# QI2lab/ray_trace_pb

Measured on NVIDIA B200. Metric: ray_surfaces_per_s_fp64, higher is better.
Workload: dtype f64

## Files before the change

ray_trace_pb_b200/csrc/rtb_device.cuh:

```cuda
#pragma once

#include <cstdint>
#include <cuda_runtime.h>

#include "../../include/rtb.h"

namespace rtb {

constexpr int kMaxSurfaces = RTB_MAX_SURFACES;
constexpr int kMaxMedia = RTB_MAX_SURFACES + 1;
constexpr int kMaxWavelengths = RTB_MAX_WAVELENGTHS;
constexpr int kMaxSlabs = 2 * RTB_MAX_SURFACES + 1;

#ifndef RTB_TRACE_THREADS
#define RTB_TRACE_THREADS 128
#endif
constexpr int kTraceThreads = RTB_TRACE_THREADS;
#ifndef RTB_TRACE_MIN_BLOCKS
#define RTB_TRACE_MIN_BLOCKS 7
#endif
constexpr int kTraceMinBlocks = RTB_TRACE_MIN_BLOCKS;

struct DevSurface {
    double cx, cy, cz;
    double nx, ny, nz;
    double ax, ay, az;
    double radius, radius_sq, abs_radius;
    double aperture;
    double focal_len;
    double nfx, nfy, nfz;
    double sin_alpha;
    double ap_sq_max;
    double on_sq_lo, on_sq_hi;
    int32_t kind;
    int8_t z_normal;
    int8_t z_axis;
    int8_t degenerate_hint;
    int8_t pad;
};

struct DevMaterial {
    double b0, b1, b2;
    double c0, c1, c2;
    double n_const;
    int32_t kind;
    int32_t pad;
};

struct DevReduce {
    double ox, oy, oz;
    double e1x, e1y, e1z;
    double e2x, e2y, e2z;
    double phase_ref;
    double half_width;
    double inv_cell;
    double *stats;
    double *grid;
    int32_t slab;
    int32_t grid_n;
    double *grid_sin;
    double *grid_count;
    double grid_n_f;
};

__host__ __device__ inline void finish_reduce(DevReduce &r)
{
    const long long plane = (long long)r.grid_n * r.grid_n;
    r.grid_sin = r.grid ? r.grid + plane : nullptr;
    r.grid_count = r.grid ? r.grid + 2 * plane : nullptr;
    r.grid_n_f = (double)r.grid_n;
}

struct DevSource {
    double a_start, a_step, a_stop;
    double b_start, b_step, b_stop;
    double px, py, pz;
    double axx, axy, axz;
    double e1x, e1y, e1z;
    double e2x, e2y, e2z;
    double wavelength;
    long long n_a, n_b;
    long long first;
    int32_t kind;
    int32_t pad;
};

struct TraceParams {
    const double *rays_in;
    double *out;
    long long n_rays;
    long long out_stride;
    int32_t n_surf;
    int32_t n_wl;
    int32_t store_last_only;
    int32_t any_store;
    int32_t flags;
    int32_t pad0;
    int16_t slab_pos[kMaxSlabs + 3];
    uint8_t slab_act[kMaxSurfaces];
    DevReduce red;
    DevSource src;
    const DevSource *src_list;
    int32_t n_src;
    int32_t pad1;
    const unsigned *lean_counts;
    unsigned long long lean_general;
    long long lean_probe_stride;
    long long lean_probe_total;
    int32_t lean_n_runs;
    int32_t lean_sample_run;
    int32_t lean_pure;
    int32_t lean_pad;
    uint8_t lean_run_end[kMaxSurfaces + 2];
    uint8_t lean_run_code[kMaxSurfaces + 2];
    DevSurface surf[kMaxSurfaces];
    DevMaterial mat[kMaxMedia];
    double wl[kMaxWavelengths];
    double n_tab[(kMaxWavelengths + 1) * kMaxMedia];
    double ratio_tab[(kMaxWavelengths + 1) * kMaxMedia];
};

static_assert(sizeof(TraceParams) < 32764, "TraceParams must fit the kernel parameter space");

__device__ __forceinline__ void ld256_stream(const double *p, double &a, double &b, double &c, double &d)
{
    asm volatile("ld.global.nc.L1::no_allocate.v4.f64 {%0,%1,%2,%3}, [%4];"
                 : "=d"(a), "=d"(b), "=d"(c), "=d"(d)
                 : "l"(p));
}

__device__ __forceinline__ void st256(double *p, double a, double b, double c, double d)
{
    asm volatile("st.global.v4.f64 [%0], {%1,%2,%3,%4};" ::"l"(p), "d"(a), "d"(b), "d"(c), "d"(d) : "memory");
}

}
```

ray_trace_pb_b200/csrc/trace_lean.cu:

```cuda
#include <cmath>
#include <math_constants.h>

#include "exact_math.cuh"
#include "lean_steps.cuh"
#include "rtb_device.cuh"
#include "surface_steps.cuh"
#include "trace_common.cuh"

namespace rtb {

namespace {

#ifndef RTB_LEAN_THREADS
#define RTB_LEAN_THREADS 128
#endif
#ifndef RTB_LEAN_MIN_BLOCKS
#define RTB_LEAN_MIN_BLOCKS 7
#endif
constexpr int kLeanThreads = RTB_LEAN_THREADS;
constexpr int kLeanMinBlocks = RTB_LEAN_MIN_BLOCKS;
constexpr int kProbeRays = 2048;
constexpr unsigned kProbeOneIn = 200;

enum StepCode : int { kLeanSphere = 0, kLeanFlat = 1, kGeneralRefracting = 2, kGeneralMirror = 3, kGeneralLens = 4,
                      kMixedRun = 5, kLeanFlatAny = 6, kLeanLens = 7, kLeanFlatZ = 8 };

__host__ __device__ inline int step_code(const DevSurface &s, bool general)
{
    const int fallback = (s.kind == RTB_SURF_MIRROR) ? kGeneralMirror
                                                     : (s.kind == RTB_SURF_PERFECT_LENS) ? kGeneralLens : kGeneralRefracting;
    if (s.kind == RTB_SURF_FLAT && s.z_axis != 0 && s.z_normal != 0) return general ? kLeanFlatZ : kLeanFlat;
    if (general) return fallback;
    if (s.kind == RTB_SURF_SPHERE) return s.z_axis != 0 ? kLeanSphere : fallback;
    if (s.kind == RTB_SURF_FLAT) return kLeanFlatAny;
    if (s.kind == RTB_SURF_PERFECT_LENS) return kLeanLens;
    return fallback;
}

__host__ __device__ inline bool has_lean_step(const DevSurface &s) { return step_code(s, false) < kGeneralRefracting || step_code(s, false) > kMixedRun; }

struct __align__(16) SurfaceShared {
    double rcp;
    int code;
    int rcp_ok;
};

struct LeanShared {
    SurfaceShared surf[kMaxSurfaces];
    int run_clean[kMaxSurfaces + 2];
};

template <bool USE_TABLE>
static __device__ __noinline__ void redo_ray(const TraceParams *P, Ray cur, int k_sample, bool sample_at, Ray *final_row,
                                             Ray *sample_row)
{
    const int n_med = P->n_surf + 1;
    const double wl0 = cur.wl;
    int row = 0;
    bool unlisted = false;
    if (USE_TABLE) {
        row = P->n_wl;
        const long long bits = __double_as_longlong(wl0);
        for (int k = 0; k < P->n_wl; k++)
            if (__double_as_longlong(P->wl[k]) == bits) row = k;
        unlisted = (row == P->n_wl) && (wl0 == wl0);
        row *= n_med;
    }
    auto index_of = [&](int medium) {
        return !USE_TABLE ? eval_index(P->mat[medium], wl0)
                          : (unlisted ? index_for_unlisted(&P->mat[medium], wl0) : P->n_tab[row + medium]);
    };
    double n1 = index_of(0);
    bool dead = false;
    Ray blank;
    set_nan(blank);
    *sample_row = blank;
    for (int k = 0; k < P->n_surf; k++) {
        if (!dead) {
            const DevSurface *s = &P->surf[k];
            const double n2 = index_of(k + 1);
            StepResult res;
            if (s->kind == RTB_SURF_FLAT || s->kind == RTB_SURF_SPHERE) {
                const double ratio = (USE_TABLE && !unlisted) ? P->ratio_tab[row + k] : xm::div(n1, n2);
                res = careful_refracting(s, cur, n1, ratio, true);
            } else if (s->kind == RTB_SURF_MIRROR) {
                res = careful_mirror(s, cur, n1);
            } else {
                res = careful_lens(s, cur, n1, n2, false);
            }
            if (k == k_sample && sample_at) *sample_row = res.at;
            cur = res.after;
            dead = res.dead;
            n1 = n2;
        }
        if (k == k_sample && !sample_at) *sample_row = dead ? blank : cur;
    }
    *final_row = dead ? blank : cur;
}

__device__ __forceinline__ void accumulate(const DevReduce &R, double ox, double oy, double oz, double phase, double *tally)
{
    const double px = ox - R.ox, py = oy - R.oy, pz = oz - R.oz;
    const double u = dot3(px, py, pz, R.e1x, R.e1y, R.e1z);
    const double v = dot3(px, py, pz, R.e2x, R.e2y, R.e2z);
    const double ph = phase - R.phase_ref;
    if (!(isfinite(u) && isfinite(v) && isfinite(ph))) return;
    if (R.stats) {
        double2 *t = reinterpret_cast<double2 *>(tally) + threadIdx.x;
        constexpr int W = kLeanThreads;
        double2 a = t[0 * W], b = t[1 * W], c = t[2 * W], d = t[3 * W], e = t[4 * W], f = t[5 * W];
        a.x += 1.0;
        a.y += u;
        b.x += v;
        b.y += u * u;
        c.x += v * v;
        c.y += u * v;
        d.x += ph;
        d.y += ph * ph;
        e.x = u < e.x ? u : e.x;
        e.y = u > e.y ? u : e.y;
        f.x = v < f.x ? v : f.x;
        f.y = v > f.y ? v : f.y;
        t[0 * W] = a; t[1 * W] = b; t[2 * W] = c; t[3 * W] = d; t[4 * W] = e; t[5 * W] = f;
    }
    if (R.grid) {
        const double xu = (u + R.half_width) * R.inv_cell;
        const double xv = (v + R.half_width) * R.inv_cell;
        const double g = R.grid_n_f;
        if (xu >= 0.0 && xu < g && xv >= 0.0 && xv < g) {
            const unsigned cell = (unsigned)__double2int_rz(xv) * (unsigned)R.grid_n + (unsigned)__double2int_rz(xu);
            double s, c;
            sincos(ph, &s, &c);
            asm volatile("red.global.add.f64 [%0], %1;" ::"l"(R.grid + cell), "d"(c) : "memory");
            asm volatile("red.global.add.f64 [%0], %1;" ::"l"(R.grid_sin + cell), "d"(s) : "memory");
            asm volatile("red.global.add.f64 [%0], %1;" ::"l"(R.grid_count + cell), "d"(1.0) : "memory");
        }
    }
}

__device__ __forceinline__ int tally_index(int k, int thread) { return ((k >> 1) * kLeanThreads + thread) * 2 + (k & 1); }

__device__ __noinline__ void flush_tally(const DevReduce &R, const double *tally)
{
    if (!R.stats) return;
    __shared__ double part[12][kLeanThreads / 32];
    const int lane = threadIdx.x & 31, warp = threadIdx.x >> 5;
    for (int k = 0; k < 12; k++) {
        double x = tally[tally_index(k, threadIdx.x)];
        x = (k < 8) ? warp_sum(x) : ((k == 8 || k == 10) ? warp_min(x) : warp_max(x));
        if (lane == 0) part[k][warp] = x;
    }
    __syncthreads();
    if (threadIdx.x < 12) {
        const int k = threadIdx.x;
        double x = part[k][0];
        for (int w = 1; w < kLeanThreads / 32; w++)
            x = (k < 8) ? x + part[k][w] : ((k == 8 || k == 10) ? fmin(x, part[k][w]) : fmax(x, part[k][w]));
        if (k < 8) {
            if (x != 0.0) atomicAdd(R.stats + k, x);
        } else if (k == 8 || k == 10) {
            if (x < CUDART_INF) atomic_min_f64(R.stats + k, x);
        } else {
            if (x > -CUDART_INF) atomic_max_f64(R.stats + k, x);
        }
    }
}

__device__ __forceinline__ bool general_step(const DevSurface &s, int code, double rcp_y, bool rcp_ok, lean::State &r, double n1,
                                             double n2, double ratio, double wl0, double wl_rcp, bool &ok, bool &kill)
{
    OptimisticZ m;
    xm::Rcp rcp_wl, rcp_k;
    rcp_wl.b = wl0; rcp_wl.y = wl_rcp; rcp_wl.ok = true;
    rcp_k.b = (code == kGeneralLens) ? s.focal_len : s.radius;
    rcp_k.y = rcp_y;
    rcp_k.ok = rcp_ok;
    Ray in, after;
    in.ox = r.ox; in.oy = r.oy; in.oz = r.oz; in.dx = r.dx; in.dy = r.dy; in.dz = r.dz; in.ph = r.ph;
    in.wl = wl0;
    AtRaw raw;
    bool dead;
    if (code == kGeneralRefracting)
        dead = refracting_step<OptimisticZ, true>(m, s, in, n1, ratio, rcp_wl, rcp_k, true, raw, after);
    else if (code == kGeneralMirror)
        dead = mirror_step<OptimisticZ, true>(m, s, in, n1, rcp_wl, raw, after);
    else
        dead = perfect_lens_step<OptimisticZ>(m, s, in, n1, n2, rcp_wl, rcp_k, false, false, raw, after);
    ok = m.ok;
    kill = raw.kill;
    r.ox = after.ox; r.oy = after.oy; r.oz = after.oz;
    r.dx = after.dx; r.dy = after.dy; r.dz = after.dz;
    r.ph = after.ph;
    return !dead;
}

template <bool USE_TABLE, bool FROM_SOURCE, bool SWEEP, bool PROBE, int KINDS>
__global__ void __launch_bounds__(kLeanThreads, kLeanMinBlocks) trace_lean_kernel(const __grid_constant__ TraceParams P,
                                                                                  unsigned *probe_counts)
{
    static_assert(!SWEEP || FROM_SOURCE, "sweeps generate their rays");
    extern __shared__ __align__(16) double s_dyn[];
    const int n_med = P.n_surf + 1;
    double *const s_pair = s_dyn;
    double *const s_tally = s_dyn + (USE_TABLE ? 2 * (P.n_wl + 1) * n_med : 0);
    __shared__ LeanShared s_c;
    __shared__ SweepShared<SWEEP> s_sweep;
    if (SWEEP) sweep_setup(P, s_sweep);
    if (USE_TABLE) {
        const int count = (P.n_wl + 1) * n_med;
        for (int k = threadIdx.x; k < count; k += blockDim.x) {
            s_pair[2 * k] = P.n_tab[k];
            s_pair[2 * k + 1] = P.ratio_tab[k];
        }
    }
    const bool reducing = !PROBE && P.red.slab >= 0;
    if (reducing && P.red.stats) {
        for (int k = 0; k < 12; k++)
            s_tally[tally_index(k, threadIdx.x)] = (k < 8) ? 0.0 : ((k == 8 || k == 10) ? CUDART_INF : -CUDART_INF);
    }
    for (int k = threadIdx.x; k < P.n_surf; k += blockDim.x) {
        const DevSurface &s = P.surf[k];
        const double den = (s.kind == RTB_SURF_PERFECT_LENS) ? s.focal_len : s.radius;
        const double rcp = xm::refine_rcp(den);
        const bool sane = xm::den_ok(den) && fabs(den) < 4503599627370496.0 && xm::quo_ok(rcp);
        s_c.surf[k].rcp = rcp;
        s_c.surf[k].rcp_ok = sane;
        bool general = ((P.lean_general >> k) & 1ull) != 0 ||
                       (!sane && (s.kind == RTB_SURF_SPHERE || s.kind == RTB_SURF_PERFECT_LENS));
        if (!PROBE && KINDS < 2 && P.lean_counts) {
            const unsigned *cnt = P.lean_counts + ((size_t)(SWEEP ? blockIdx.y : 0) * kMaxSurfaces + k) * 2;
            general |= (unsigned long long)cnt[1] * kProbeOneIn > (unsigned long long)cnt[0];
        }
        s_c.surf[k].code = step_code(s, general);
    }
    __syncthreads();
    for (int run = threadIdx.x; KINDS < 2 && run < P.lean_n_runs; run += blockDim.x) {
        bool clean = true;
        for (int k = run > 0 ? P.lean_run_end[run - 1] : 0; k < P.lean_run_end[run]; k++)
            clean &= s_c.surf[k].code == P.lean_run_code[run];
        s_c.run_clean[run] = clean;
    }
    __syncthreads();

    const DevSource &source = sweep_source(P, s_sweep);
    const DevReduce &red = sweep_reduce(P, s_sweep);
    const long long row0 = SWEEP ? (long long)blockIdx.y * P.n_rays : 0;
    const int k_red = reducing ? ((P.red.slab - 1) >> 1) : -1;
    const bool sample_at = reducing && (P.red.slab & 1) != 0;
    const bool planes_in = (P.flags & RTB_FLAG_PLANES_IN) != 0, planes_out = (P.flags & RTB_FLAG_PLANES_OUT) != 0;
    const long long out_rows = P.out_stride / 8;
    const long long stride = (long long)gridDim.x * blockDim.x;
    unsigned *const my_counts = PROBE ? probe_counts + (size_t)(SWEEP ? blockIdx.y : 0) * kMaxSurfaces * 2 : nullptr;

    for (long long base = (long long)blockIdx.x * blockDim.x; base < P.n_rays; base += stride) {
        long long i = base + threadIdx.x;
        const bool valid = i < P.n_rays;
        if (PROBE) {
            const long long st = P.lean_probe_stride;
            i = i * st + (long long)((unsigned)(i * 2654435761u) % (unsigned long long)st);
            if (i >= P.lean_probe_total) i = P.lean_probe_total - 1;
        }
        Ray cur;
        set_nan(cur);
        if (valid) {
            if (FROM_SOURCE)
                cur = make_ray(source, source.first + i);
            else
                load_ray(P.rays_in, i, PROBE ? P.lean_probe_total : P.n_rays, planes_in, cur);
        }
        const double wl0 = cur.wl;
        const double wl_rcp = xm::refine_rcp(wl0);
        int row = 0;
        bool listed = true;
        if (USE_TABLE) {
            row = P.n_wl;
            const long long bits = __double_as_longlong(wl0);
#pragma unroll 1
            for (int k = 0; k < P.n_wl; k++)
                if (__double_as_longlong(P.wl[k]) == bits) row = k;
            listed = row != P.n_wl;
        }
        const double *pair = s_pair + 2 * row * n_med;
        auto non_finite = [](double v) { return (__double2hiint(v) & 0x7ff00000) == 0x7ff00000; };
        const unsigned wl_exp = ((unsigned)__double2hiint(wl0) >> 20) & 0x7ffu;
        const bool fit = valid && listed && (wl_exp - 923u <= 200u) &&
                         !(non_finite(cur.ox) | non_finite(cur.oy) | non_finite(cur.oz) | non_finite(cur.dx) |
                           non_finite(cur.dy) | non_finite(cur.dz) | non_finite(cur.ph));
        bool failed = valid && !fit;
        bool alive = fit;
        bool sampled = false, at_valid = false;
        lean::State r = {cur.ox, cur.oy, cur.oz, cur.dx, cur.dy, cur.dz, cur.ph};
        double n1 = 0.0;
        if (!USE_TABLE) n1 = eval_index(P.mat[0], wl0);

        if (!PROBE) {
            for (int run = 0; run < P.lean_n_runs; run++) {
                const int begin = run > 0 ? P.lean_run_end[run - 1] : 0;
                const int end = P.lean_run_end[run];
                const int code = (KINDS >= 2 || s_c.run_clean[run]) ? P.lean_run_code[run] : kMixedRun;
                if (code == kLeanSphere) {
                    for (int k = begin; k < end; k++) {
                        if (!__any_sync(0xffffffffu, alive)) {
                            at_valid = false;
                            break;
                        }
                        if (USE_TABLE) {
                            n1 = pair[0];
                            pair += 2;
                        }
                        const double n2 = USE_TABLE ? 0.0 : eval_index(P.mat[k + 1], wl0);
                        const double ratio = USE_TABLE ? pair[-1] : xm::div(n1, n2);
                        bool ok = true, kill;
                        const bool on = lean::sphere_axial(ok, P.surf[k], s_c.surf[k].rcp, r, n1, ratio, wl0, wl_rcp, kill);
                        failed = failed | (alive & !ok);
                        at_valid = alive & ok & !kill;
                        alive = alive & ok & on;
                        if (!USE_TABLE) n1 = n2;
                    }
                } else if (code == kLeanFlat) {
                    for (int k = begin; k < end; k++) {
                        if (!__any_sync(0xffffffffu, alive)) {
                            at_valid = false;
                            break;
                        }
                        if (USE_TABLE) {
                            n1 = pair[0];
                            pair += 2;
                        }
                        const double n2 = USE_TABLE ? 0.0 : eval_index(P.mat[k + 1], wl0);
                        const double ratio = USE_TABLE ? pair[-1] : xm::div(n1, n2);
                        bool ok = true, kill;
                        const bool on = lean::flat_axial<false>(ok, P.surf[k], r, n1, ratio, wl0, wl_rcp, kill);
                        failed = failed | (alive & !ok);
                        at_valid = alive & ok & !kill;
                        alive = alive & ok & on;
                        if (!USE_TABLE) n1 = n2;
                    }
                } else if (KINDS >= 2 && code == kLeanFlatZ) {
                    for (int k = begin; k < end; k++) {
                        if (!__any_sync(0xffffffffu, alive)) {
                            at_valid = false;
                            break;
                        }
                        if (USE_TABLE) {
                            n1 = pair[0];
                            pair += 2;
                        }
                        const double n2 = USE_TABLE ? 0.0 : eval_index(P.mat[k + 1], wl0);
                        const double ratio = USE_TABLE ? pair[-1] : xm::div(n1, n2);
                        bool ok = true, kill;
                        const bool on = lean::flat_axial<true>(ok, P.surf[k], r, n1, ratio, wl0, wl_rcp, kill);
                        failed = failed | (alive & !ok);
                        at_valid = alive & ok & !kill;
                        alive = alive & ok & on;
                        if (!USE_TABLE) n1 = n2;
                    }
                } else if ((KINDS == 1 || KINDS == 3) && code == kLeanFlatAny) {
                    for (int k = begin; k < end; k++) {
                        if (!__any_sync(0xffffffffu, alive)) {
                            at_valid = false;
                            break;
                        }
                        if (USE_TABLE) {
                            n1 = pair[0];
                            pair += 2;
                        }
                        const double n2 = USE_TABLE ? 0.0 : eval_index(P.mat[k + 1], wl0);
                        const double ratio = USE_TABLE ? pair[-1] : xm::div(n1, n2);
                        bool ok = true, kill;
                        const bool on = lean::flat_any(ok, P.surf[k], r, n1, ratio, wl0, wl_rcp, kill);
                        failed = failed | (alive & !ok);
                        at_valid = alive & ok & !kill;
                        alive = alive & ok & on;
                        if (!USE_TABLE) n1 = n2;
                    }
                } else if ((KINDS == 1 || KINDS == 3) && code == kLeanLens) {
                    for (int k = begin; k < end; k++) {
                        if (!__any_sync(0xffffffffu, alive)) {
                            at_valid = false;
                            break;
                        }
                        double n2;
                        if (USE_TABLE) {
                            n1 = pair[0];
                            n2 = pair[2];
                            pair += 2;
                        } else {
                            n2 = eval_index(P.mat[k + 1], wl0);
                        }
                        bool ok = true;
                        const bool on = lean::lens_any(ok, P.surf[k], s_c.surf[k].rcp, r, n1, n2, wl0, wl_rcp);
                        failed = failed | (alive & !ok);
                        at_valid = false;
                        alive = alive & ok & on;
                        if (!USE_TABLE) n1 = n2;
                    }
                } else if (KINDS == 1 && code == kGeneralLens) {
                    for (int k = begin; k < end; k++) {
                        if (!__any_sync(0xffffffffu, alive)) {
                            at_valid = false;
                            break;
                        }
                        const DevSurface &s = P.surf[k];
                        const SurfaceShared ss = s_c.surf[k];
                        double ratio, n2;
                        if (USE_TABLE) {
                            n1 = pair[0];
                            ratio = pair[1];
                            n2 = pair[2];
                            pair += 2;
                        } else {
                            n2 = eval_index(P.mat[k + 1], wl0);
                            ratio = xm::div(n1, n2);
                        }
                        bool ok = true, kill;
                        const bool on = general_step(s, kGeneralLens, ss.rcp, ss.rcp_ok != 0, r, n1, n2, ratio, wl0, wl_rcp, ok, kill);
                        failed = failed | (alive & !ok);
                        at_valid = alive & ok & !kill;
                        alive = alive & ok & on;
                        if (!USE_TABLE) n1 = n2;
                    }
                } else if (KINDS < 2 && code == kGeneralRefracting) {
                    for (int k = begin; k < end; k++) {
                        if (!__any_sync(0xffffffffu, alive)) {
                            at_valid = false;
                            break;
                        }
                        const DevSurface &s = P.surf[k];
                        const SurfaceShared ss = s_c.surf[k];
                        double ratio, n2 = 0.0;
                        if (USE_TABLE) {
                            n1 = pair[0];
                            ratio = pair[1];
                            pair += 2;
                        } else {
                            n2 = eval_index(P.mat[k + 1], wl0);
                            ratio = xm::div(n1, n2);
                        }
                        bool ok = true, kill;
                        const bool on = general_step(s, kGeneralRefracting, ss.rcp, ss.rcp_ok != 0, r, n1, n2, ratio, wl0, wl_rcp, ok, kill);
                        failed = failed | (alive & !ok);
                        at_valid = alive & ok & !kill;
                        alive = alive & ok & on;
                        if (!USE_TABLE) n1 = n2;
                    }
                } else if (KINDS < 2) {
                    for (int k = begin; k < end; k++) {
                        if (!__any_sync(0xffffffffu, alive)) {
                            at_valid = false;
                            break;
                        }
                        const DevSurface &s = P.surf[k];
                        const SurfaceShared ss = s_c.surf[k];
                        double ratio, n2 = 0.0;
                        if (USE_TABLE) {
                            n1 = pair[0];
                            ratio = pair[1];
                            n2 = pair[2];
                            pair += 2;
                        } else {
                            n2 = eval_index(P.mat[k + 1], wl0);
                            ratio = xm::div(n1, n2);
                        }
                        bool ok = true, kill;
                        bool on;
                        if (ss.code == kLeanSphere) {
                            on = lean::sphere_axial(ok, s, ss.rcp, r, n1, ratio, wl0, wl_rcp, kill);
                        } else if (ss.code == kLeanFlat) {
                            on = lean::flat_axial<false>(ok, s, r, n1, ratio, wl0, wl_rcp, kill);
                        } else if (ss.code == kLeanFlatZ) {
                            on = lean::flat_axial<true>(ok, s, r, n1, ratio, wl0, wl_rcp, kill);
                        } else if (KINDS == 1 && ss.code == kLeanFlatAny) {
                            on = lean::flat_any(ok, s, r, n1, ratio, wl0, wl_rcp, kill);
                        } else if (KINDS == 1 && ss.code == kLeanLens) {
                            on = lean::lens_any(ok, s, ss.rcp, r, n1, n2, wl0, wl_rcp);
                            kill = false;
                        } else {
                            on = general_step(s, KINDS == 1 ? ss.code : (int)kGeneralRefracting, ss.rcp, ss.rcp_ok != 0, r, n1,
                                              n2, ratio, wl0, wl_rcp, ok, kill);
                        }
                        failed = failed | (alive & !ok);
                        at_valid = alive & ok & !kill;
                        alive = alive & ok & on;
                        if (!USE_TABLE) n1 = n2;
                    }
                }
                if (run == P.lean_sample_run && (sample_at ? at_valid : alive)) {
                    accumulate(red, r.ox, r.oy, r.oz, r.ph, s_tally);
                    sampled = true;
                }
            }
        } else {
            for (int k = 0; k < P.n_surf; k++) {
                if (!alive) break;
                const DevSurface &s = P.surf[k];
                const SurfaceShared ss = s_c.surf[k];
                const int code = ss.code;
                double ratio, n2;
                if (USE_TABLE) {
                    n1 = pair[0];
                    ratio = pair[1];
                    n2 = pair[2];
                    pair += 2;
                } else {
                    n2 = eval_index(P.mat[k + 1], wl0);
                    ratio = xm::div(n1, n2);
                }
                const lean::State before = r;
                bool ok = true, on, kill;
                if (code == kLeanSphere)
                    on = lean::sphere_axial(ok, s, ss.rcp, r, n1, ratio, wl0, wl_rcp, kill);
                else if (code == kLeanFlat)
                    on = lean::flat_axial<false>(ok, s, r, n1, ratio, wl0, wl_rcp, kill);
                else if (code == kLeanFlatZ)
                    on = lean::flat_axial<true>(ok, s, r, n1, ratio, wl0, wl_rcp, kill);
                else if (code == kLeanFlatAny)
                    on = lean::flat_any(ok, s, r, n1, ratio, wl0, wl_rcp, kill);
                else if (code == kLeanLens)
                    on = lean::lens_any(ok, s, ss.rcp, r, n1, n2, wl0, wl_rcp);
                else
                    on = general_step(s, code, ss.rcp, ss.rcp_ok != 0, r, n1, n2, ratio, wl0, wl_rcp, ok, kill);
                atomicAdd(my_counts + 2 * k, 1u);
                if (!ok) {
                    atomicAdd(my_counts + 2 * k + 1, 1u);
                    Ray in;
                    in.ox = before.ox; in.oy = before.oy; in.oz = before.oz;
                    in.dx = before.dx; in.dy = before.dy; in.dz = before.dz;
                    in.ph = before.ph; in.wl = wl0;
                    StepResult res;
                    if (s.kind == RTB_SURF_FLAT || s.kind == RTB_SURF_SPHERE)
                        res = careful_refracting(&s, in, n1, ratio, true);
                    else if (s.kind == RTB_SURF_MIRROR)
                        res = careful_mirror(&s, in, n1);
                    else
                        res = careful_lens(&s, in, n1, n2, false);
                    r.ox = res.after.ox; r.oy = res.after.oy; r.oz = res.after.oz;
                    r.dx = res.after.dx; r.dy = res.after.dy; r.dz = res.after.dz;
                    r.ph = res.after.ph;
                    on = !res.dead;
                }
                alive = on;
                if (!USE_TABLE) n1 = n2;
            }
        }
        if (PROBE) continue;

        Ray out;
        out.ox = r.ox; out.oy = r.oy; out.oz = r.oz; out.dx = r.dx; out.dy = r.dy; out.dz = r.dz; out.ph = r.ph;
        out.wl = wl0;
        if (!alive) set_nan(out);
        if (failed) {
            Ray launch, sample, redone;
            if (FROM_SOURCE)
                launch = make_ray(source, source.first + i);
            else
                load_ray(P.rays_in, i, P.n_rays, planes_in, launch);
            redo_ray<USE_TABLE>(&P, launch, k_red, sample_at, &redone, &sample);
            out = redone;
            if (reducing && !sampled) accumulate(red, sample.ox, sample.oy, sample.oz, sample.ph, s_tally);
        }
        if (valid && P.any_store) store_ray(P.out, row0 + i, out_rows, planes_out, out);
    }
    if (reducing) flush_tally(red, s_tally);
}

bool refracting_only(const TraceParams &P)
{
    for (int k = 0; k < P.n_surf; k++) {
        const DevSurface &s = P.surf[k];
        if (!(s.kind == RTB_SURF_SPHERE || (s.kind == RTB_SURF_FLAT && s.z_axis != 0 && s.z_normal != 0))) return false;
    }
    return true;
}

template <bool T, bool S, bool W, bool PR>
cudaError_t launch_lean_one(const TraceParams &P, unsigned blocks, unsigned n_y, unsigned *probe_counts, cudaStream_t stream)
{
    size_t dyn = T ? 2 * sizeof(double) * (size_t)(P.n_wl + 1) * (size_t)(P.n_surf + 1) : 0;
    if (!PR && P.red.slab >= 0 && P.red.stats) dyn += sizeof(double) * 12 * kLeanThreads;
    const bool pure = !PR && P.lean_pure != 0;
    static const bool loaded = [] {
        cudaFuncAttributes a;
        cudaFuncGetAttributes(&a, trace_lean_kernel<T, S, W, false, 0>);
        cudaFuncGetAttributes(&a, trace_lean_kernel<T, S, W, false, 1>);
        cudaFuncGetAttributes(&a, trace_lean_kernel<T, S, W, false, 2>);
        cudaFuncGetAttributes(&a, trace_lean_kernel<T, S, W, false, 3>);
        cudaFuncGetAttributes(&a, trace_lean_kernel<T, S, W, true, 1>);
        cudaGetLastError();
        return true;
    }();
    (void)loaded;
    if (pure && refracting_only(P))
        trace_lean_kernel<T, S, W, false, 2><<<dim3(blocks, n_y), kLeanThreads, dyn, stream>>>(P, probe_counts);
    else if (pure)
        trace_lean_kernel<T, S, W, false, 3><<<dim3(blocks, n_y), kLeanThreads, dyn, stream>>>(P, probe_counts);
    else if (!PR && refracting_only(P))
        trace_lean_kernel<T, S, W, PR, 0><<<dim3(blocks, n_y), kLeanThreads, dyn, stream>>>(P, probe_counts);
    else
        trace_lean_kernel<T, S, W, PR, 1><<<dim3(blocks, n_y), kLeanThreads, dyn, stream>>>(P, probe_counts);
    return cudaGetLastError();
}

template <bool PR>
cudaError_t launch_lean_pick(const TraceParams &P, unsigned blocks, unsigned *probe_counts, cudaStream_t stream)
{
    const bool table = P.n_wl > 0, source = P.src.kind >= 0, sweep = P.n_src > 0;
    const unsigned n_y = sweep ? (unsigned)P.n_src : 1u;
#ifdef RTB_LEAN_ONLY_ONE
    return launch_lean_one<true, false, false, PR>(P, blocks, 1, probe_counts, stream);
#endif
    if (sweep)
        return table ? launch_lean_one<true, true, true, PR>(P, blocks, n_y, probe_counts, stream)
                     : launch_lean_one<false, true, true, PR>(P, blocks, n_y, probe_counts, stream);
    if (table)
        return source ? launch_lean_one<true, true, false, PR>(P, blocks, 1, probe_counts, stream)
                      : launch_lean_one<true, false, false, PR>(P, blocks, 1, probe_counts, stream);
    return source ? launch_lean_one<false, true, false, PR>(P, blocks, 1, probe_counts, stream)
                  : launch_lean_one<false, false, false, PR>(P, blocks, 1, probe_counts, stream);
}

}

int g_lean_min_share_pct = 75;
void set_lean_min_share_pct(int pct) { g_lean_min_share_pct = pct; }

bool lean_eligible(const TraceParams &P)
{
    if (P.flags & RTB_FLAG_INTERSECT_ONLY) return false;
    if (P.any_store && !P.store_last_only) return false;
    if (P.red.slab == 0) return false;
    if (P.red.slab > 0 && (P.red.slab & 1) != 0 && P.surf[(P.red.slab - 1) >> 1].kind == RTB_SURF_PERFECT_LENS) return false;
    int n_lean = 0;
    for (int k = 0; k < P.n_surf; k++) {
        const DevSurface &s = P.surf[k];
        n_lean += has_lean_step(s);
    }
    if (100 * n_lean < g_lean_min_share_pct * P.n_surf) return false;
    if (P.red.slab < 0 && !P.any_store) return false;
    return P.n_surf > 0;
}

unsigned long long lean_verdict_from_counts(const unsigned *counts, int n_src, int n_surf)
{
    unsigned long long general = 0ull;
    for (int j = 0; j < n_src; j++)
        for (int k = 0; k < n_surf; k++) {
            const unsigned *cnt = counts + ((size_t)j * kMaxSurfaces + k) * 2;
            if ((unsigned long long)cnt[1] * kProbeOneIn > (unsigned long long)cnt[0]) general |= 1ull << k;
        }
    return general;
}

namespace {
bool sane_reciprocal(const DevSurface &s)
{
    const double den = (s.kind == RTB_SURF_PERFECT_LENS) ? s.focal_len : s.radius;
    const bool needs_rcp = s.kind == RTB_SURF_SPHERE || s.kind == RTB_SURF_PERFECT_LENS;
    return !needs_rcp || (std::isfinite(den) && fabs(den) > 1e-150 && fabs(den) < 4503599627370496.0);
}

bool build_runs(TraceParams &P, unsigned long long general)
{
    const int k_red = P.red.slab >= 0 ? (P.red.slab - 1) >> 1 : -1;
    bool all_lean = P.n_surf > 0;
    P.lean_n_runs = 0;
    P.lean_sample_run = -1;
    int prev = -1;
    for (int k = 0; k < P.n_surf; k++) {
        const DevSurface &s = P.surf[k];
        const int code = step_code(s, ((general >> k) & 1ull) != 0 || !sane_reciprocal(s));
        all_lean &= code < kGeneralRefracting || code > kMixedRun;
        if (code != prev) P.lean_n_runs++;
        P.lean_run_code[P.lean_n_runs - 1] = (uint8_t)code;
        P.lean_run_end[P.lean_n_runs - 1] = (uint8_t)(k + 1);
        prev = code;
        if (k == k_red) {
            P.lean_sample_run = P.lean_n_runs - 1;
            prev = -1;
        }
    }
    return all_lean;
}
}

cudaError_t launch_trace_lean(const TraceParams &P_in, unsigned *counts, int sm_count, cudaStream_t stream, int *launches,
                              int pure_mode, unsigned long long verdict_general, bool *pure_used, bool probe_optional,
                              bool *probed)
{
    if (pure_used) *pure_used = false;
    if (probed) *probed = false;
    if (P_in.n_rays <= 0) return cudaSuccess;
    TraceParams P = P_in;
    const bool sweep = P.n_src > 0;
    const int n_sources = sweep ? P.n_src : 1;
    P.lean_general = 0ull;
    for (int k = 0; k < P.n_surf; k++) {
        const DevSurface &s = P.surf[k];
        if (!has_lean_step(s)) P.lean_general |= 1ull << k;
    }
    P.lean_pure = 0;
    if (pure_mode != 0 && P.lean_general == 0ull && build_runs(P, pure_mode == 1 ? verdict_general : 0ull))
        P.lean_pure = 1;
    else
        build_runs(P, P.lean_general);
    if (pure_used) *pure_used = P.lean_pure != 0;
    if (P.lean_pure != 0 && probe_optional) counts = nullptr;
    if (probed) *probed = counts != nullptr;
    cudaError_t e;
    P.lean_counts = nullptr;
    if (counts) {
        e = cudaMemsetAsync(counts, 0, sizeof(unsigned) * 2 * kMaxSurfaces * (size_t)n_sources, stream);
        if (e != cudaSuccess) return e;
        TraceParams Q = P;
        const long long n_probe = P.n_rays < kProbeRays ? P.n_rays : kProbeRays;
        Q.lean_probe_total = P.n_rays;
        Q.lean_probe_stride = P.n_rays / n_probe;
        Q.n_rays = n_probe;
        Q.red.slab = -1;
        Q.any_store = 0;
        const unsigned pb = (unsigned)((n_probe + kLeanThreads - 1) / kLeanThreads);
        e = launch_lean_pick<true>(Q, pb, counts, stream);
        if (e != cudaSuccess) return e;
        if (launches) ++*launches;
        P.lean_counts = counts;
    }
    long long blocks = (P.n_rays + kLeanThreads - 1) / kLeanThreads;
    long long max_blocks = (long long)sm_count * kLeanMinBlocks * 4;
    if (sweep) max_blocks = (max_blocks + P.n_src - 1) / P.n_src;
    if (blocks > max_blocks) blocks = max_blocks;
    e = launch_lean_pick<false>(P, (unsigned)blocks, nullptr, stream);
    if (e == cudaSuccess && launches) ++*launches;
    return e;
}

}
```

Baseline: 79.31 billion.

## Add one-wavelength lean kernel variants, axis-frame fast accumulate, split sample leg

New measurement: 80.32 billion (median of 6 runs). +1.3%, better.

```diff
diff --git a/ray_trace_pb_b200/csrc/rtb_device.cuh b/ray_trace_pb_b200/csrc/rtb_device.cuh
--- a/ray_trace_pb_b200/csrc/rtb_device.cuh
+++ b/ray_trace_pb_b200/csrc/rtb_device.cuh
@@ -1,6 +1,7 @@
 #pragma once
 
 #include <cstdint>
+#include <cstring>
 #include <cuda_runtime.h>
 
 #include "../../include/rtb.h"
@@ -61,6 +62,8 @@
     double *grid_sin;
     double *grid_count;
     double grid_n_f;
+    int32_t axis_frame;
+    int32_t pad;
 };
 
 __host__ __device__ inline void finish_reduce(DevReduce &r)
@@ -69,6 +72,14 @@
     r.grid_sin = r.grid ? r.grid + plane : nullptr;
     r.grid_count = r.grid ? r.grid + 2 * plane : nullptr;
     r.grid_n_f = (double)r.grid_n;
+    auto bits = [](double x) {
+        unsigned long long b;
+        memcpy(&b, &x, sizeof b);
+        return b;
+    };
+    constexpr unsigned long long kOne = 0x3ff0000000000000ull;
+    r.axis_frame = bits(r.e1x) == kOne && bits(r.e1y) == 0 && bits(r.e1z) == 0 && bits(r.e2x) == 0 &&
+                   bits(r.e2y) == kOne && bits(r.e2z) == 0;
 }
 
 struct DevSource {
diff --git a/ray_trace_pb_b200/csrc/trace_lean.cu b/ray_trace_pb_b200/csrc/trace_lean.cu
--- a/ray_trace_pb_b200/csrc/trace_lean.cu
+++ b/ray_trace_pb_b200/csrc/trace_lean.cu
@@ -101,10 +101,20 @@
 __device__ __forceinline__ void accumulate(const DevReduce &R, double ox, double oy, double oz, double phase, double *tally)
 {
     const double px = ox - R.ox, py = oy - R.oy, pz = oz - R.oz;
-    const double u = dot3(px, py, pz, R.e1x, R.e1y, R.e1z);
-    const double v = dot3(px, py, pz, R.e2x, R.e2y, R.e2z);
     const double ph = phase - R.phase_ref;
-    if (!(isfinite(u) && isfinite(v) && isfinite(ph))) return;
+    double u, v;
+    if (R.axis_frame) {
+        const unsigned hx = __double2hiint(px), hy = __double2hiint(py), hz = __double2hiint(pz), hp = __double2hiint(ph);
+        const double z = __hiloint2double((int)(hx & hy & hz & 0x80000000u), 0);
+        u = px + z;
+        v = py + z;
+        const unsigned top = max(max(hx & 0x7fffffffu, hy & 0x7fffffffu), max(hz & 0x7fffffffu, hp & 0x7fffffffu));
+        if (top >= 0x7ff00000u) return;
+    } else {
+        u = dot3(px, py, pz, R.e1x, R.e1y, R.e1z);
+        v = dot3(px, py, pz, R.e2x, R.e2y, R.e2z);
+        if (!(isfinite(u) && isfinite(v) && isfinite(ph))) return;
+    }
     if (R.stats) {
         double2 *t = reinterpret_cast<double2 *>(tally) + threadIdx.x;
         constexpr int W = kLeanThreads;
@@ -194,11 +204,12 @@
     return !dead;
 }
 
-template <bool USE_TABLE, bool FROM_SOURCE, bool SWEEP, bool PROBE, int KINDS>
+template <bool USE_TABLE, bool FROM_SOURCE, bool SWEEP, bool PROBE, int KINDS, bool ONE_ROW = false>
 __global__ void __launch_bounds__(kLeanThreads, kLeanMinBlocks) trace_lean_kernel(const __grid_constant__ TraceParams P,
                                                                                   unsigned *probe_counts)
 {
     static_assert(!SWEEP || FROM_SOURCE, "sweeps generate their rays");
+    static_assert(!ONE_ROW || (USE_TABLE && !PROBE && KINDS >= 2), "one-row forms of the pure table kernels only");
     extern __shared__ __align__(16) double s_dyn[];
     const int n_med = P.n_surf + 1;
     double *const s_pair = s_dyn;
@@ -206,7 +217,7 @@
     __shared__ LeanShared s_c;
     __shared__ SweepShared<SWEEP> s_sweep;
     if (SWEEP) sweep_setup(P, s_sweep);
-    if (USE_TABLE) {
+    if (USE_TABLE && !ONE_ROW) {
         const int count = (P.n_wl + 1) * n_med;
         for (int k = threadIdx.x; k < count; k += blockDim.x) {
             s_pair[2 * k] = P.n_tab[k];
@@ -251,6 +262,7 @@
     const long long out_rows = P.out_stride / 8;
     const long long stride = (long long)gridDim.x * blockDim.x;
     unsigned *const my_counts = PROBE ? probe_counts + (size_t)(SWEEP ? blockIdx.y : 0) * kMaxSurfaces * 2 : nullptr;
+    const double wl_rcp_one = (USE_TABLE && (ONE_ROW || P.n_wl == 1)) ? xm::refine_rcp(P.wl[0]) : 0.0;
 
     for (long long base = (long long)blockIdx.x * blockDim.x; base < P.n_rays; base += stride) {
         long long i = base + threadIdx.x;
@@ -268,24 +280,31 @@
             else
                 load_ray(P.rays_in, i, PROBE ? P.lean_probe_total : P.n_rays, planes_in, cur);
         }
-        const double wl0 = cur.wl;
-        const double wl_rcp = xm::refine_rcp(wl0);
+        const double wl_ray = cur.wl;
+        double wl_rcp;
         int row = 0;
         bool listed = true;
-        if (USE_TABLE) {
-            row = P.n_wl;
-            const long long bits = __double_as_longlong(wl0);
+        if (USE_TABLE && (ONE_ROW || P.n_wl == 1)) {
+            listed = __double_as_longlong(wl_ray) == __double_as_longlong(P.wl[0]);
+            wl_rcp = wl_rcp_one;
+        } else {
+            wl_rcp = xm::refine_rcp(wl_ray);
+            if (USE_TABLE) {
+                row = P.n_wl;
+                const long long bits = __double_as_longlong(wl_ray);
 #pragma unroll 1
-            for (int k = 0; k < P.n_wl; k++)
-                if (__double_as_longlong(P.wl[k]) == bits) row = k;
-            listed = row != P.n_wl;
+                for (int k = 0; k < P.n_wl; k++)
+                    if (__double_as_longlong(P.wl[k]) == bits) row = k;
+                listed = row != P.n_wl;
+            }
         }
         const double *pair = s_pair + 2 * row * n_med;
-        auto non_finite = [](double v) { return (__double2hiint(v) & 0x7ff00000) == 0x7ff00000; };
-        const unsigned wl_exp = ((unsigned)__double2hiint(wl0) >> 20) & 0x7ffu;
-        const bool fit = valid && listed && (wl_exp - 923u <= 200u) &&
-                         !(non_finite(cur.ox) | non_finite(cur.oy) | non_finite(cur.oz) | non_finite(cur.dx) |
-                           non_finite(cur.dy) | non_finite(cur.dz) | non_finite(cur.ph));
+        auto mag = [](double v) { return (unsigned)__double2hiint(v) & 0x7fffffffu; };
+        const unsigned top = max(max(max(mag(cur.ox), mag(cur.oy)), max(mag(cur.oz), mag(cur.dx))),
+                                 max(max(mag(cur.dy), mag(cur.dz)), mag(cur.ph)));
+        const unsigned wl_exp = ((unsigned)__double2hiint(wl_ray) >> 20) & 0x7ffu;
+        const bool fit = valid && listed && (wl_exp - 923u <= 200u) && top < 0x7ff00000u;
+        const double wl0 = ONE_ROW ? P.wl[0] : wl_ray;
         bool failed = valid && !fit;
         bool alive = fit;
         bool sampled = false, at_valid = false;
@@ -294,198 +313,214 @@
         if (!USE_TABLE) n1 = eval_index(P.mat[0], wl0);
 
         if (!PROBE) {
-            for (int run = 0; run < P.lean_n_runs; run++) {
-                const int begin = run > 0 ? P.lean_run_end[run - 1] : 0;
-                const int end = P.lean_run_end[run];
-                const int code = (KINDS >= 2 || s_c.run_clean[run]) ? P.lean_run_code[run] : kMixedRun;
-                if (code == kLeanSphere) {
-                    for (int k = begin; k < end; k++) {
-                        if (!__any_sync(0xffffffffu, alive)) {
+            int run = 0;
+#pragma unroll 1
+            for (int leg = 0; leg < 2; leg++) {
+                const int leg_end = leg == 0 ? P.lean_sample_run + 1 : P.lean_n_runs;
+                for (; run < leg_end; run++) {
+                    const int begin = run > 0 ? P.lean_run_end[run - 1] : 0;
+                    const int end = P.lean_run_end[run];
+                    const int code = (KINDS >= 2 || s_c.run_clean[run]) ? P.lean_run_code[run] : kMixedRun;
+                    if (code == kLeanSphere) {
+                        for (int k = begin; k < end; k++) {
+                            if (!__any_sync(0xffffffffu, alive)) {
+                                at_valid = false;
+                                break;
+                            }
+                            if (ONE_ROW) {
+                                n1 = P.n_tab[k];
+                            } else if (USE_TABLE) {
+                                n1 = pair[0];
+                                pair += 2;
+                            }
+                            const double n2 = USE_TABLE ? 0.0 : eval_index(P.mat[k + 1], wl0);
+                            const double ratio = ONE_ROW ? P.ratio_tab[k] : USE_TABLE ? pair[-1] : xm::div(n1, n2);
+                            bool ok = true, kill;
+                            const bool on = lean::sphere_axial(ok, P.surf[k], s_c.surf[k].rcp, r, n1, ratio, wl0, wl_rcp, kill);
+                            failed = failed | (alive & !ok);
+                            at_valid = alive & ok & !kill;
+                            alive = alive & ok & on;
+                            if (!USE_TABLE) n1 = n2;
+                        }
+                    } else if (code == kLeanFlat) {
+                        for (int k = begin; k < end; k++) {
+                            if (!__any_sync(0xffffffffu, alive)) {
+                                at_valid = false;
+                                break;
+                            }
+                            if (ONE_ROW) {
+                                n1 = P.n_tab[k];
+                            } else if (USE_TABLE) {
+                                n1 = pair[0];
+                                pair += 2;
+                            }
+                            const double n2 = USE_TABLE ? 0.0 : eval_index(P.mat[k + 1], wl0);
+                            const double ratio = ONE_ROW ? P.ratio_tab[k] : USE_TABLE ? pair[-1] : xm::div(n1, n2);
+                            bool ok = true, kill;
+                            const bool on = lean::flat_axial<false>(ok, P.surf[k], r, n1, ratio, wl0, wl_rcp, kill);
+                            failed = failed | (alive & !ok);
+                            at_valid = alive & ok & !kill;
+                            alive = alive & ok & on;
+                            if (!USE_TABLE) n1 = n2;
+                        }
+                    } else if (KINDS >= 2 && code == kLeanFlatZ) {
+                        for (int k = begin; k < end; k++) {
+                            if (!__any_sync(0xffffffffu, alive)) {
+                                at_valid = false;
+                                break;
+                            }
+                            if (ONE_ROW) {
+                                n1 = P.n_tab[k];
+                            } else if (USE_TABLE) {
+                                n1 = pair[0];
+                                pair += 2;
+                            }
+                            const double n2 = USE_TABLE ? 0.0 : eval_index(P.mat[k + 1], wl0);
+                            const double ratio = ONE_ROW ? P.ratio_tab[k] : USE_TABLE ? pair[-1] : xm::div(n1, n2);
+                            bool ok = true, kill;
+                            const bool on = lean::flat_axial<true>(ok, P.surf[k], r, n1, ratio, wl0, wl_rcp, kill);
+                            failed = failed | (alive & !ok);
+                            at_valid = alive & ok & !kill;
+                            alive = alive & ok & on;
+                            if (!USE_TABLE) n1 = n2;
+                        }
+                    } else if ((KINDS == 1 || KINDS == 3) && code == kLeanFlatAny) {
+                        for (int k = begin; k < end; k++) {
+                            if (!__any_sync(0xffffffffu, alive)) {
+                                at_valid = false;
+                                break;
+                            }
+                            if (ONE_ROW) {
+                                n1 = P.n_tab[k];
+                            } else if (USE_TABLE) {
+                                n1 = pair[0];
+                                pair += 2;
+                            }
+                            const double n2 = USE_TABLE ? 0.0 : eval_index(P.mat[k + 1], wl0);
+                            const double ratio = ONE_ROW ? P.ratio_tab[k] : USE_TABLE ? pair[-1] : xm::div(n1, n2);
+                            bool ok = true, kill;
+                            const bool on = lean::flat_any(ok, P.surf[k], r, n1, ratio, wl0, wl_rcp, kill);
+                            failed = failed | (alive & !ok);
+                            at_valid = alive & ok & !kill;
+                            alive = alive & ok & on;
+                            if (!USE_TABLE) n1 = n2;
+                        }
+                    } else if ((KINDS == 1 || KINDS == 3) && code == kLeanLens) {
+                        for (int k = begin; k < end; k++) {
+                            if (!__any_sync(0xffffffffu, alive)) {
+                                at_valid = false;
+                                break;
+                            }
+                            double n2;
+                            if (ONE_ROW) {
+                                n1 = P.n_tab[k];
+                                n2 = P.n_tab[k + 1];
+                            } else if (USE_TABLE) {
+                                n1 = pair[0];
+                                n2 = pair[2];
+                                pair += 2;
+                            } else {
+                                n2 = eval_index(P.mat[k + 1], wl0);
+                            }
+                            bool ok = true;
+                            const bool on = lean::lens_any(ok, P.surf[k], s_c.surf[k].rcp, r, n1, n2, wl0, wl_rcp);
+                            failed = failed | (alive & !ok);
                             at_valid = false;
-                            break;
+                            alive = alive & ok & on;
+                            if (!USE_TABLE) n1 = n2;
                         }
-                        if (USE_TABLE) {
-                            n1 = pair[0];
-                            pair += 2;
+                    } else if (KINDS == 1 && code == kGeneralLens) {
+                        for (int k = begin; k < end; k++) {
+                            if (!__any_sync(0xffffffffu, alive)) {
+                                at_valid = false;
+                                break;
+                            }
+                            const DevSurface &s = P.surf[k];
+                            const SurfaceShared ss = s_c.surf[k];
+                            double ratio, n2;
+                            if (USE_TABLE) {
+                                n1 = pair[0];
+                                ratio = pair[1];
+                                n2 = pair[2];
+                                pair += 2;
+                            } else {
+                                n2 = eval_index(P.mat[k + 1], wl0);
+                                ratio = xm::div(n1, n2);
+                            }
+                            bool ok = true, kill;
+                            const bool on = general_step(s, kGeneralLens, ss.rcp, ss.rcp_ok != 0, r, n1, n2, ratio, wl0, wl_rcp, ok, kill);
+                            failed = failed | (alive & !ok);
+                            at_valid = alive & ok & !kill;
+                            alive = alive & ok & on;
+                            if (!USE_TABLE) n1 = n2;
                         }
-                        const double n2 = USE_TABLE ? 0.0 : eval_index(P.mat[k + 1], wl0);
-                        const double ratio = USE_TABLE ? pair[-1] : xm::div(n1, n2);
-                        bool ok = true, kill;
-                        const bool on = lean::sphere_axial(ok, P.surf[k], s_c.surf[k].rcp, r, n1, ratio, wl0, wl_rcp, kill);
-                        failed = failed | (alive & !ok);
-                        at_valid = alive & ok & !kill;
-                        alive = alive & ok & on;
-                        if (!USE_TABLE) n1 = n2;
-                    }
-                } else if (code == kLeanFlat) {
-                    for (int k = begin; k < end; k++) {
-                        if (!__any_sync(0xffffffffu, alive)) {
-                            at_valid = false;
-                            break;
+                    } else if (KINDS < 2 && code == kGeneralRefracting) {
+                        for (int k = begin; k < end; k++) {
+                            if (!__any_sync(0xffffffffu, alive)) {
+                                at_valid = false;
+                                break;
+                            }
+                            const DevSurface &s = P.surf[k];
+                            const SurfaceShared ss = s_c.surf[k];
+                            double ratio, n2 = 0.0;
+                            if (USE_TABLE) {
+                                n1 = pair[0];
+                                ratio = pair[1];
+                                pair += 2;
+                            } else {
+                                n2 = eval_index(P.mat[k + 1], wl0);
+                                ratio = xm::div(n1, n2);
+                            }
+                            bool ok = true, kill;
+                            const bool on = general_step(s, kGeneralRefracting, ss.rcp, ss.rcp_ok != 0, r, n1, n2, ratio, wl0, wl_rcp, ok, kill);
+                            failed = failed | (alive & !ok);
+                            at_valid = alive & ok & !kill;
+                            alive = alive & ok & on;
+                            if (!USE_TABLE) n1 = n2;
                         }
-                        if (USE_TABLE) {
-                            n1 = pair[0];
-                            pair += 2;
+                    } else if (KINDS < 2) {
+                        for (int k = begin; k < end; k++) {
+                            if (!__any_sync(0xffffffffu, alive)) {
+                                at_valid = false;
+                                break;
+                            }
+                            const DevSurface &s = P.surf[k];
+                            const SurfaceShared ss = s_c.surf[k];
+                            double ratio, n2 = 0.0;
+                            if (USE_TABLE) {
+                                n1 = pair[0];
+                                ratio = pair[1];
+                                n2 = pair[2];
+                                pair += 2;
+                            } else {
+                                n2 = eval_index(P.mat[k + 1], wl0);
+                                ratio = xm::div(n1, n2);
+                            }
+                            bool ok = true, kill;
+                            bool on;
+                            if (ss.code == kLeanSphere) {
+                                on = lean::sphere_axial(ok, s, ss.rcp, r, n1, ratio, wl0, wl_rcp, kill);
+                            } else if (ss.code == kLeanFlat) {
+                                on = lean::flat_axial<false>(ok, s, r, n1, ratio, wl0, wl_rcp, kill);
+                            } else if (ss.code == kLeanFlatZ) {
+                                on = lean::flat_axial<true>(ok, s, r, n1, ratio, wl0, wl_rcp, kill);
+                            } else if (KINDS == 1 && ss.code == kLeanFlatAny) {
+                                on = lean::flat_any(ok, s, r, n1, ratio, wl0, wl_rcp, kill);
+                            } else if (KINDS == 1 && ss.code == kLeanLens) {
+                                on = lean::lens_any(ok, s, ss.rcp, r, n1, n2, wl0, wl_rcp);
+                                kill = false;
+                            } else {
+                                on = general_step(s, KINDS == 1 ? ss.code : (int)kGeneralRefracting, ss.rcp, ss.rcp_ok != 0,
+                                                  r, n1, n2, ratio, wl0, wl_rcp, ok, kill);
+                            }
+                            failed = failed | (alive & !ok);
+                            at_valid = alive & ok & !kill;
+                            alive = alive & ok & on;
+                            if (!USE_TABLE) n1 = n2;
                         }
-                        const double n2 = USE_TABLE ? 0.0 : eval_index(P.mat[k + 1], wl0);
-                        const double ratio = USE_TABLE ? pair[-1] : xm::div(n1, n2);
-                        bool ok = true, kill;
-                        const bool on = lean::flat_axial<false>(ok, P.surf[k], r, n1, ratio, wl0, wl_rcp, kill);
-                        failed = failed | (alive & !ok);
-                        at_valid = alive & ok & !kill;
-                        alive = alive & ok & on;
-                        if (!USE_TABLE) n1 = n2;
-                    }
-                } else if (KINDS >= 2 && code == kLeanFlatZ) {
-                    for (int k = begin; k < end; k++) {
-                        if (!__any_sync(0xffffffffu, alive)) {
-                            at_valid = false;
-                            break;
-                        }
-                        if (USE_TABLE) {
-                            n1 = pair[0];
-                            pair += 2;
-                        }
-                        const double n2 = USE_TABLE ? 0.0 : eval_index(P.mat[k + 1], wl0);
-                        const double ratio = USE_TABLE ? pair[-1] : xm::div(n1, n2);
-                        bool ok = true, kill;
-                        const bool on = lean::flat_axial<true>(ok, P.surf[k], r, n1, ratio, wl0, wl_rcp, kill);
-                        failed = failed | (alive & !ok);
-                        at_valid = alive & ok & !kill;
-                        alive = alive & ok & on;
-                        if (!USE_TABLE) n1 = n2;
-                    }
-                } else if ((KINDS == 1 || KINDS == 3) && code == kLeanFlatAny) {
-                    for (int k = begin; k < end; k++) {
-                        if (!__any_sync(0xffffffffu, alive)) {
-                            at_valid = false;
-                            break;
-                        }
-                        if (USE_TABLE) {
-                            n1 = pair[0];
-                            pair += 2;
-                        }
-                        const double n2 = USE_TABLE ? 0.0 : eval_index(P.mat[k + 1], wl0);
-                        const double ratio = USE_TABLE ? pair[-1] : xm::div(n1, n2);
-                        bool ok = true, kill;
-                        const bool on = lean::flat_any(ok, P.surf[k], r, n1, ratio, wl0, wl_rcp, kill);
-                        failed = failed | (alive & !ok);
-                        at_valid = alive & ok & !kill;
-                        alive = alive & ok & on;
-                        if (!USE_TABLE) n1 = n2;
-                    }
-                } else if ((KINDS == 1 || KINDS == 3) && code == kLeanLens) {
-                    for (int k = begin; k < end; k++) {
-                        if (!__any_sync(0xffffffffu, alive)) {
-                            at_valid = false;
-                            break;
-                        }
-                        double n2;
-                        if (USE_TABLE) {
-                            n1 = pair[0];
-                            n2 = pair[2];
-                            pair += 2;
-                        } else {
-                            n2 = eval_index(P.mat[k + 1], wl0);
-                        }
-                        bool ok = true;
-                        const bool on = lean::lens_any(ok, P.surf[k], s_c.surf[k].rcp, r, n1, n2, wl0, wl_rcp);
-                        failed = failed | (alive & !ok);
-                        at_valid = false;
-                        alive = alive & ok & on;
-                        if (!USE_TABLE) n1 = n2;
-                    }
-                } else if (KINDS == 1 && code == kGeneralLens) {
-                    for (int k = begin; k < end; k++) {
-                        if (!__any_sync(0xffffffffu, alive)) {
-                            at_valid = false;
-                            break;
-                        }
-                        const DevSurface &s = P.surf[k];
-                        const SurfaceShared ss = s_c.surf[k];
-                        double ratio, n2;
-                        if (USE_TABLE) {
-                            n1 = pair[0];
-                            ratio = pair[1];
-                            n2 = pair[2];
-                            pair += 2;
-                        } else {
-                            n2 = eval_index(P.mat[k + 1], wl0);
-                            ratio = xm::div(n1, n2);
-                        }
-                        bool ok = true, kill;
-                        const bool on = general_step(s, kGeneralLens, ss.rcp, ss.rcp_ok != 0, r, n1, n2, ratio, wl0, wl_rcp, ok, kill);
-                        failed = failed | (alive & !ok);
-                        at_valid = alive & ok & !kill;
-                        alive = alive & ok & on;
-                        if (!USE_TABLE) n1 = n2;
-                    }
-                } else if (KINDS < 2 && code == kGeneralRefracting) {
-                    for (int k = begin; k < end; k++) {
-                        if (!__any_sync(0xffffffffu, alive)) {
-                            at_valid = false;
-                            break;
-                        }
-                        const DevSurface &s = P.surf[k];
-                        const SurfaceShared ss = s_c.surf[k];
-                        double ratio, n2 = 0.0;
-                        if (USE_TABLE) {
-                            n1 = pair[0];
-                            ratio = pair[1];
-                            pair += 2;
-                        } else {
-                            n2 = eval_index(P.mat[k + 1], wl0);
-                            ratio = xm::div(n1, n2);
-                        }
-                        bool ok = true, kill;
-                        const bool on = general_step(s, kGeneralRefracting, ss.rcp, ss.rcp_ok != 0, r, n1, n2, ratio, wl0, wl_rcp, ok, kill);
-                        failed = failed | (alive & !ok);
-                        at_valid = alive & ok & !kill;
-                        alive = alive & ok & on;
-                        if (!USE_TABLE) n1 = n2;
-                    }
-                } else if (KINDS < 2) {
-                    for (int k = begin; k < end; k++) {
-                        if (!__any_sync(0xffffffffu, alive)) {
-                            at_valid = false;
-                            break;
-                        }
-                        const DevSurface &s = P.surf[k];
-                        const SurfaceShared ss = s_c.surf[k];
-                        double ratio, n2 = 0.0;
-                        if (USE_TABLE) {
-                            n1 = pair[0];
-                            ratio = pair[1];
-                            n2 = pair[2];
-                            pair += 2;
-                        } else {
-                            n2 = eval_index(P.mat[k + 1], wl0);
-                            ratio = xm::div(n1, n2);
-                        }
-                        bool ok = true, kill;
-                        bool on;
-                        if (ss.code == kLeanSphere) {
-                            on = lean::sphere_axial(ok, s, ss.rcp, r, n1, ratio, wl0, wl_rcp, kill);
-                        } else if (ss.code == kLeanFlat) {
-                            on = lean::flat_axial<false>(ok, s, r, n1, ratio, wl0, wl_rcp, kill);
-                        } else if (ss.code == kLeanFlatZ) {
-                            on = lean::flat_axial<true>(ok, s, r, n1, ratio, wl0, wl_rcp, kill);
-                        } else if (KINDS == 1 && ss.code == kLeanFlatAny) {
-                            on = lean::flat_any(ok, s, r, n1, ratio, wl0, wl_rcp, kill);
-                        } else if (KINDS == 1 && ss.code == kLeanLens) {
-                            on = lean::lens_any(ok, s, ss.rcp, r, n1, n2, wl0, wl_rcp);
-                            kill = false;
-                        } else {
-                            on = general_step(s, KINDS == 1 ? ss.code : (int)kGeneralRefracting, ss.rcp, ss.rcp_ok != 0, r, n1,
-                                              n2, ratio, wl0, wl_rcp, ok, kill);
-                        }
-                        failed = failed | (alive & !ok);
-                        at_valid = alive & ok & !kill;
-                        alive = alive & ok & on;
-                        if (!USE_TABLE) n1 = n2;
                     }
                 }
-                if (run == P.lean_sample_run && (sample_at ? at_valid : alive)) {
+                if (leg == 0 && reducing && (sample_at ? at_valid : alive)) {
                     accumulate(red, r.ox, r.oy, r.oz, r.ph, s_tally);
                     sampled = true;
                 }
@@ -585,12 +620,19 @@
         cudaFuncGetAttributes(&a, trace_lean_kernel<T, S, W, false, 1>);
         cudaFuncGetAttributes(&a, trace_lean_kernel<T, S, W, false, 2>);
         cudaFuncGetAttributes(&a, trace_lean_kernel<T, S, W, false, 3>);
+        cudaFuncGetAttributes(&a, trace_lean_kernel<T, S, W, false, 2, T>);
+        cudaFuncGetAttributes(&a, trace_lean_kernel<T, S, W, false, 3, T>);
         cudaFuncGetAttributes(&a, trace_lean_kernel<T, S, W, true, 1>);
         cudaGetLastError();
         return true;
     }();
     (void)loaded;
-    if (pure && refracting_only(P))
+    const bool one_row = T && P.n_wl == 1;
+    if (pure && one_row && refracting_only(P))
+        trace_lean_kernel<T, S, W, false, 2, T><<<dim3(blocks, n_y), kLeanThreads, dyn, stream>>>(P, probe_counts);
+    else if (pure && one_row)
+        trace_lean_kernel<T, S, W, false, 3, T><<<dim3(blocks, n_y), kLeanThreads, dyn, stream>>>(P, probe_counts);
+    else if (pure && refracting_only(P))
         trace_lean_kernel<T, S, W, false, 2><<<dim3(blocks, n_y), kLeanThreads, dyn, stream>>>(P, probe_counts);
     else if (pure)
         trace_lean_kernel<T, S, W, false, 3><<<dim3(blocks, n_y), kLeanThreads, dyn, stream>>>(P, probe_counts);
```
